# Kim-Dongjun/Soft-Truncation

Measured on AMD Instinct MI355X. Metric: training images/sec (DDPM++ CIFAR-10 32x32), higher is better.
Workload: dtype f32; 1 GPU; DDPM++ (VP) CIFAR-10 32x32, configs/vp/CIFAR10/ddpmpp_nll_st.py (BASELINE configs[1]); per_gpu_batch=128, global_batch=128, parallelism=dp1

## Files before the change

soft-truncation_amd/csrc/conv_x2w.h:

```cpp
#pragma once

namespace x2w {

typedef short s4 __attribute__((__vector_size__(8)));
typedef __attribute__((address_space(3))) s4 lds_s4;
typedef __attribute__((address_space(3))) void lds_void;

struct Args {
  const unsigned char* dypl; const float* dyrec; long dy_ps;
  const unsigned char* xpl; const float* xrec; long x_ps;
  float* part; long part_stride;
  int N, H, W, HW, Cin, Cout, Cob, Cib;
  int tiles_co, tiles_ci, nchunks_total, chunks_per_split;
};

__device__ __forceinline__ halfx8 cat(s4 lo, s4 hi) {
  typedef short s8 __attribute__((__vector_size__(16)));
  const s8 v = __builtin_shufflevector(lo, hi, 0, 1, 2, 3, 4, 5, 6, 7);
  return __builtin_bit_cast(halfx8, v);
}

constexpr int A_INSTR = 3;
constexpr int A_BLK = A_INSTR * 16 * 64;
constexpr int A_PLANE = 4 * A_BLK;
constexpr int B_INSTR = 6;
constexpr int B_PLANE = B_INSTR * 16 * 64;
constexpr int BUF = 2 * A_PLANE + 2 * B_PLANE;

constexpr int X1_FORM = 16;
template <int COLS, int FORM = 1>
__global__ __launch_bounds__(256 * (FORM & 15), 2) void wgrad_kernel(Args a) {
  constexpr int GROUPS = FORM & 15;
  constexpr bool X1 = (FORM & X1_FORM) != 0;
  constexpr int NS = X1 ? 1 : 2;
  constexpr int STAGES = 2;
  constexpr bool TWO = COLS == 4;
  constexpr int ROWS = 32 / COLS;
  constexpr int TPA = COLS + 2;
  constexpr int TRB = TWO ? 12 : ROWS + 2;
  constexpr int LDS = STAGES * BUF;
  static_assert(ROWS * TPA <= A_INSTR * 16 && TRB * COLS <= B_INSTR * 16, "tiles exceed the staged slots");
  __shared__ __attribute__((aligned(1024))) unsigned char lds_all[LDS * GROUPS];
  const int tid = threadIdx.x & 255, lane = tid & 63;
  const int grp = GROUPS == 1 ? 0 : __builtin_amdgcn_readfirstlane((int)threadIdx.x >> 8);
  const int wid = __builtin_amdgcn_readfirstlane(tid >> 6);
  unsigned char* const lds = lds_all + grp * LDS;
  __shared__ float red_amax[2][GROUPS][4];
  x2::LateAmax amax_dy, amax_x;
  amax_dy.load(a.dyrec, x2::NPART, tid);
  amax_x.load(a.xrec, x2::NPART, tid);
  const int ntiles = a.tiles_co * a.tiles_ci;
  const int id = xcd_remap(blockIdx.x, gridDim.x);
  const int tile = id % ntiles, zs = id / ntiles;
  const int tco = tile % a.tiles_co, tci = tile / a.tiles_co;
  const int co_blk = tco * 4 + wid;
  const bool co_live = co_blk < a.Cob;
  const int c_begin = zs * a.chunks_per_split;
  const int c_last = min(a.nchunks_total, c_begin + a.chunks_per_split) - 1;

  const __amdgpu_buffer_rsrc_t a_rs = x2::make_rsrc(a.dypl, 2L * a.dy_ps);
  const __amdgpu_buffer_rsrc_t b_rs = x2::make_rsrc(a.xpl, 2L * a.x_ps);
  const int piece = (lane & 3) * 16;
  int a_rel[A_INSTR], a_c[A_INSTR];
#pragma unroll
  for (int j = 0; j < A_INSTR; ++j) {
    const int sl = 16 * j + (lane >> 2);
    int r = sl / TPA;
    a_c[j] = sl - r * TPA;
    int img = 0;
    if (TWO) { img = r >> 2; r &= 3; }
    if (sl >= ROWS * TPA || !co_live) a_c[j] = -1000000;
    a_rel[j] = (img * a.Cob * a.HW + r * a.W + a_c[j] - 1) * 64 + piece;
  }
  int b_rel[3], b_ty[3], b_dst[3]; unsigned b_pl[3];
#pragma unroll
  for (int u = 0; u < 3; ++u) {
    const int idx = wid + 4 * u, j = idx % B_INSTR, pl = idx / B_INSTR;
    const int sl = 16 * j + (lane >> 2);
    b_ty[u] = sl / COLS;
    const int tx = sl - b_ty[u] * COLS;
    int img = 0;
    if (TWO) { img = b_ty[u] / 6; b_ty[u] -= 6 * img; }
    if (sl >= TRB * COLS) b_ty[u] = -1000000;
    b_rel[u] = (img * a.Cib * a.HW + (b_ty[u] - 1) * a.W + tx) * 64 + piece;
    b_dst[u] = 2 * A_PLANE + pl * B_PLANE + j * 1024;
    b_pl[u] = (unsigned)pl;
  }
  auto stage = [&](int c, unsigned char* buf) {
    const int p0 = c * 32;
    const int b = p0 / a.HW, hw0 = p0 - b * a.HW;
    const int y0 = hw0 / a.W, x0 = hw0 - y0 * a.W;
    const int a_chunk = ((b * a.Cob + co_blk) * a.HW + hw0) * 64;
#pragma unroll
    for (int j = 0; j < A_INSTR; ++j) {
      const int xx = x0 + a_c[j] - 1;
      const unsigned vo = (xx >= 0 && xx < a.W) ? (unsigned)(a_chunk + a_rel[j]) : 0x80000000u;
#pragma unroll
      for (int s = 0; s < NS; ++s)
        __builtin_amdgcn_raw_ptr_buffer_load_lds(a_rs, (lds_void*)(buf + s * A_PLANE + wid * A_BLK + j * 1024), 16,
                                                 (int)vo, (int)(s * (unsigned)a.dy_ps), 0, 0);
    }
    const int b_chunk = ((b * a.Cib + tci) * a.HW + hw0) * 64;
#pragma unroll
    for (int u = 0; u < 3; ++u) {
      if (X1 && b_pl[u]) continue;
      const int yy = y0 + b_ty[u] - 1;
      const unsigned vo = (yy >= 0 && yy < a.H) ? (unsigned)(b_chunk + b_rel[u]) : 0x80000000u;
      __builtin_amdgcn_raw_ptr_buffer_load_lds(b_rs, (lds_void*)(buf + b_dst[u]), 16, (int)vo, (int)(b_pl[u] * (unsigned)a.x_ps), 0, 0);
    }
  };

  floatx16 acc[9];
#pragma unroll
  for (int t = 0; t < 9; ++t)
#pragma unroll
    for (int e = 0; e < 16; ++e) acc[t][e] = 0.f;

  const int m = lane & 15, g = lane >> 4;
  const int ch_off = (16 * (g & 1) + 4 * (m & 3)) * 2;
  int a_off[2][2], b_off[2][2];
#pragma unroll
  for (int kk = 0; kk < 2; ++kk)
#pragma unroll
    for (int h = 0; h < 2; ++h) {
      const int k = 16 * kk + 8 * (g >> 1) + 4 * h + (m >> 2);
      const int krow = k / COLS, kcol = k - krow * COLS;
      a_off[kk][h] = wid * A_BLK + (krow * TPA + kcol + 1) * 64 + ch_off;
      const int trow = TWO ? (krow >> 2) * 6 + (krow & 3) : krow;
      b_off[kk][h] = 2 * A_PLANE + ((trow + 1) * COLS + kcol) * 64 + ch_off;
    }
  constexpr int SA[3] = {1, 0, 0}, SB[3] = {0, 1, 0};

  auto compute = [&](const unsigned char* buf) {
#pragma unroll
    for (int kk = 0; kk < 2; ++kk) {
      halfx8 af[3][2];
#pragma unroll
      for (int t = 0; t < 3; ++t)
#pragma unroll
        for (int s = 0; s < NS; ++s)
          af[t][s] = cat(__builtin_amdgcn_ds_read_tr16_b64_v4i16((lds_s4*)(buf + s * A_PLANE + a_off[kk][0] - (t - 1) * 64)),
                         __builtin_amdgcn_ds_read_tr16_b64_v4i16((lds_s4*)(buf + s * A_PLANE + a_off[kk][1] - (t - 1) * 64)));
#pragma unroll
      for (int t3 = 0; t3 < 3; ++t3) {
        halfx8 bf[2];
#pragma unroll
        for (int s = 0; s < NS; ++s)
          bf[s] = cat(__builtin_amdgcn_ds_read_tr16_b64_v4i16((lds_s4*)(buf + s * B_PLANE + b_off[kk][0] + (t3 - 1) * COLS * 64)),
                      __builtin_amdgcn_ds_read_tr16_b64_v4i16((lds_s4*)(buf + s * B_PLANE + b_off[kk][1] + (t3 - 1) * COLS * 64)));
#pragma unroll
        for (int pr = X1 ? 2 : 0; pr < 3; ++pr)
#pragma unroll
          for (int t = 0; t < 3; ++t)
            acc[3 * t3 + t] = __builtin_amdgcn_mfma_f32_32x32x16_f16(af[t][SA[pr]], bf[SB[pr]], acc[3 * t3 + t], 0, 0, 0);
      }
    }
  };

  const int rounds = (c_last - c_begin + GROUPS) / GROUPS;
#pragma unroll
  for (int i = 0; i < STAGES - 1; ++i)
    if (c_begin + i * GROUPS + grp <= c_last) stage(c_begin + i * GROUPS + grp, lds + i * BUF);
  int cur = 0;
  for (int it = 0; it < rounds; ++it) {
    const int c = c_begin + it * GROUPS + grp;
    asm volatile("s_waitcnt vmcnt(0)" ::: "memory");
    __syncthreads();
    const int nxt = cur + STAGES - 1 >= STAGES ? cur - 1 : cur + STAGES - 1;
    if (c + (STAGES - 1) * GROUPS <= c_last) stage(c + (STAGES - 1) * GROUPS, lds + nxt * BUF);
    if (c <= c_last) compute(lds + cur * BUF);
    cur = cur + 1 == STAGES ? 0 : cur + 1;
  }
  const float sa = x2::pow2_scale_of(amax_dy.reduce(red_amax[0][grp], tid));
  const float sb = x2::pow2_scale_of(amax_x.reduce(red_amax[1][grp], tid));
  const float unscale = 1.f / (sa * sb);
  if (GROUPS == 2) {
    float* const xch = reinterpret_cast<float*>(lds_all);
#pragma unroll
    for (int r = 0; r < 3; ++r) {
      __syncthreads();
      if (grp == 1) {
#pragma unroll
        for (int t = 0; t < 3; ++t)
#pragma unroll
          for (int e = 0; e < 16; ++e) xch[(16 * t + e) * 256 + tid] = acc[3 * r + t][e];
      }
      __syncthreads();
      if (grp == 0) {
#pragma unroll
        for (int t = 0; t < 3; ++t)
#pragma unroll
          for (int e = 0; e < 16; ++e) acc[3 * r + t][e] += xch[(16 * t + e) * 256 + tid];
      }
    }
    if (grp == 1) return;
  }

  float* slab = a.part + (long)zs * a.part_stride;
  const int fk = lane >> 5, fc = lane & 31;
  const int ci = tci * 32 + fc;
  if (co_live && ci < a.Cin) {
#pragma unroll
    for (int t = 0; t < 9; ++t)
#pragma unroll
      for (int e = 0; e < 16; ++e) {
        const int co = co_blk * 32 + 4 * fk + igemm::strip_row(e);
        if (co < a.Cout) slab[((long)t * a.Cout + co) * a.Cin + ci] = unscale * acc[t][e];
      }
  }
}


struct Plan { int ok; int splits; int chunks_per_split; long slab; int groups; };
inline int groups_mode() { static const int v = [] { const char* e = getenv("STK_X2W_GROUPS"); return e ? atoi(e) : 2; }(); return v; }
inline Plan plan(int N, int H, int W, int Cin, int Cout, int wgs = 0) {
  Plan r = {0, 1, 0, 0, 1};
  if (H != W || W < 4 || (W & (W - 1)) || Cin % 32 || Cout % 32 || Cin < 32 || Cout < 32) return r;
  const long px = (long)N * H * W;
  if (px % 32 || px / 32 > 0x7fffffffL / 64) return r;
  const int nch = (int)(px / 32);
  const long tiles = (long)stk_cdiv(Cout, 128) * (Cin / 32);
  static const long cap_mb = [] { const char* e = getenv("STK_WGRAD_SLAB_MB"); return e ? atol(e) : 128L; }();
  static const long shared = [] { const char* e = getenv("STK_X2W_WGS"); return e && atol(e) > 0 ? atol(e) : 256L; }();
  const long target = wgs > 0 ? wgs : shared;
  long splits = tiles >= target ? 1 : target / tiles;
  if (splits > nch / 8) splits = nch / 8;
  const long cap = (cap_mb << 20) / (9L * Cout * Cin * 4);
  if (splits > cap) splits = cap;
  if (splits < 1) splits = 1;
  const bool gw = groups_mode() == 3 || (groups_mode() == 2 && (W == 8 || W == 16));
  if (gw && splits >= 2 && splits % 2 == 0 && nch / splits >= 8) { r.groups = 2; splits /= 2; }
  r.chunks_per_split = stk_cdiv(nch, splits);
  r.splits = stk_cdiv(nch, r.chunks_per_split);
  r.slab = 9L * Cout * Cin;
  r.ok = nch >= 8;
  return r;
}

}
```

Measured before the change: 3438 images/s.

## Trim wgrad LDS staging: whole-row dy loads, exact x-tile instruction count, inline-asm DMA

Rewrites the LDS staging of the fp16 weight-gradient conv kernel. When dy tiles cover whole image rows, it issues two buffer-to-LDS loads instead of three and zeroes the halo columns once up front. It also issues only the x-tile load instructions that are actually live rather than a fixed three per wave. Buffer loads now go through inline asm that sets m0 directly, and lane/tid are recomputed late (mbcnt) to shorten live ranges. The aim is less redundant global traffic and lower VGPR pressure, at the cost of fragile hand-written asm (m0 save/restore, s_nop) and extra special-case index logic.

Result: faster. 3497 images/s (median of 6 runs) (+1.7%).

```diff
diff --git a/soft-truncation_amd/csrc/conv_x2w.h b/soft-truncation_amd/csrc/conv_x2w.h
--- a/soft-truncation_amd/csrc/conv_x2w.h
+++ b/soft-truncation_amd/csrc/conv_x2w.h
@@ -18,6 +18,17 @@
   typedef short s8 __attribute__((__vector_size__(16)));
   const s8 v = __builtin_shufflevector(lo, hi, 0, 1, 2, 3, 4, 5, 6, 7);
   return __builtin_bit_cast(halfx8, v);
+}
+
+__device__ __forceinline__ u32x4 rsrc_words(const void* base, long bytes) {
+  const unsigned long p = reinterpret_cast<unsigned long>(base);
+  return u32x4{(unsigned)p, (unsigned)(p >> 32) & 0xffffu, (unsigned)bytes, 0x00020000u};
+}
+__device__ __forceinline__ void dma16(u32x4 rs, const unsigned char* dst, unsigned voff, unsigned soff) {
+  const unsigned lds_addr = (unsigned)(unsigned long)(lds_void*)dst;
+  unsigned keep;
+  asm volatile("s_mov_b32 %0, m0\n\ts_mov_b32 m0, %1\n\ts_nop 4\n\tbuffer_load_dwordx4 %2, %3, %4 offen lds\n\ts_mov_b32 m0, %0"
+               : "=&s"(keep) : "s"(lds_addr), "v"(voff), "s"(rs), "s"(soff) : "memory");
 }
 
 constexpr int A_INSTR = 3;
@@ -58,10 +69,12 @@
   const int c_begin = zs * a.chunks_per_split;
   const int c_last = min(a.nchunks_total, c_begin + a.chunks_per_split) - 1;
 
-  const __amdgpu_buffer_rsrc_t a_rs = x2::make_rsrc(a.dypl, 2L * a.dy_ps);
-  const __amdgpu_buffer_rsrc_t b_rs = x2::make_rsrc(a.xpl, 2L * a.x_ps);
+  const u32x4 a_rs = rsrc_words(a.dypl, 2L * a.dy_ps);
+  const u32x4 b_rs = rsrc_words(a.xpl, 2L * a.x_ps);
   const int piece = (lane & 3) * 16;
-  int a_rel[A_INSTR], a_c[A_INSTR];
+  const bool a_whole_rows = COLS == 16 || (COLS == 32 && a.W == 32);
+  const int a_instr = a_whole_rows ? 2 : A_INSTR;
+  int a_rel[A_INSTR], a_c[A_INSTR], a_dst[A_INSTR];
 #pragma unroll
   for (int j = 0; j < A_INSTR; ++j) {
     const int sl = 16 * j + (lane >> 2);
@@ -69,15 +82,24 @@
     a_c[j] = sl - r * TPA;
     int img = 0;
     if (TWO) { img = r >> 2; r &= 3; }
-    if (sl >= ROWS * TPA || !co_live) a_c[j] = -1000000;
+    if (sl >= ROWS * TPA) a_c[j] = -1000000;
     a_rel[j] = (img * a.Cob * a.HW + r * a.W + a_c[j] - 1) * 64 + piece;
-  }
-  int b_rel[3], b_ty[3], b_dst[3]; unsigned b_pl[3];
-#pragma unroll
-  for (int u = 0; u < 3; ++u) {
-    const int idx = wid + 4 * u, j = idx % B_INSTR, pl = idx / B_INSTR;
+    a_dst[j] = wid * A_BLK + j * 1024;
+    if (a_whole_rows) {
+      a_c[j] = 1;
+      a_rel[j] = sl * 64 + piece;
+      a_dst[j] = wid * A_BLK + ((16 * j / COLS) * TPA + 16 * j % COLS + 1) * 64;
+    }
+    if (!co_live) { a_c[j] = -1000000; a_rel[j] = -1000000 * 64; }
+  }
+  constexpr int B_LIVE = TRB * COLS / 16, B_ALL = NS * B_LIVE, B_WAVE = (B_ALL + 3) / 4;
+  static_assert(B_LIVE * 16 == TRB * COLS && B_LIVE <= B_INSTR, "the x tile is whole instructions");
+  int b_rel[B_WAVE], b_ty[B_WAVE], b_dst[B_WAVE]; unsigned b_pl[B_WAVE];
+#pragma unroll
+  for (int u = 0; u < B_WAVE; ++u) {
+    const int idx = wid + 4 * u, j = idx % B_LIVE, pl = idx / B_LIVE;
     const int sl = 16 * j + (lane >> 2);
-    b_ty[u] = sl / COLS;
+    b_ty[u] = COLS >= 16 ? 16 * j / COLS : sl / COLS;
     const int tx = sl - b_ty[u] * COLS;
     int img = 0;
     if (TWO) { img = b_ty[u] / 6; b_ty[u] -= 6 * img; }
@@ -93,20 +115,21 @@
     const int a_chunk = ((b * a.Cob + co_blk) * a.HW + hw0) * 64;
 #pragma unroll
     for (int j = 0; j < A_INSTR; ++j) {
+      if (j >= a_instr) continue;
       const int xx = x0 + a_c[j] - 1;
-      const unsigned vo = (xx >= 0 && xx < a.W) ? (unsigned)(a_chunk + a_rel[j]) : 0x80000000u;
+      const bool in = COLS == 32 ? (unsigned)(x0 * 64 + a_rel[j]) < (unsigned)(a.W * 64) : (xx >= 0 && xx < a.W);
+      const unsigned vo = in ? (unsigned)(a_chunk + a_rel[j]) : 0x80000000u;
 #pragma unroll
       for (int s = 0; s < NS; ++s)
-        __builtin_amdgcn_raw_ptr_buffer_load_lds(a_rs, (lds_void*)(buf + s * A_PLANE + wid * A_BLK + j * 1024), 16,
-                                                 (int)vo, (int)(s * (unsigned)a.dy_ps), 0, 0);
+        dma16(a_rs, buf + s * A_PLANE + a_dst[j], vo, s * (unsigned)a.dy_ps);
     }
     const int b_chunk = ((b * a.Cib + tci) * a.HW + hw0) * 64;
 #pragma unroll
-    for (int u = 0; u < 3; ++u) {
-      if (X1 && b_pl[u]) continue;
+    for (int u = 0; u < B_WAVE; ++u) {
+      if (4 * u + 3 >= B_ALL && wid + 4 * u >= B_ALL) continue;
       const int yy = y0 + b_ty[u] - 1;
       const unsigned vo = (yy >= 0 && yy < a.H) ? (unsigned)(b_chunk + b_rel[u]) : 0x80000000u;
-      __builtin_amdgcn_raw_ptr_buffer_load_lds(b_rs, (lds_void*)(buf + b_dst[u]), 16, (int)vo, (int)(b_pl[u] * (unsigned)a.x_ps), 0, 0);
+      dma16(b_rs, buf + b_dst[u], vo, b_pl[u] * (unsigned)a.x_ps);
     }
   };
 
@@ -158,6 +181,14 @@
   };
 
   const int rounds = (c_last - c_begin + GROUPS) / GROUPS;
+  if (a_whole_rows) {
+    constexpr int NH = COLS >= 16 ? STAGES * NS * ROWS * 2 : 0;
+    static_assert(NH * 4 <= 64, "one store per lane");
+    const int h = lane >> 2, side = h & 1, r = (h >> 1) % ROWS, sp = (h >> 1) / ROWS;
+    if (h < NH)
+      *reinterpret_cast<uint4*>(lds + (sp / NS) * BUF + (sp % NS) * A_PLANE + wid * A_BLK + (r * TPA + side * (TPA - 1)) * 64 + piece) =
+          make_uint4(0u, 0u, 0u, 0u);
+  }
 #pragma unroll
   for (int i = 0; i < STAGES - 1; ++i)
     if (c_begin + i * GROUPS + grp <= c_last) stage(c_begin + i * GROUPS + grp, lds + i * BUF);
@@ -171,8 +202,10 @@
     if (c <= c_last) compute(lds + cur * BUF);
     cur = cur + 1 == STAGES ? 0 : cur + 1;
   }
-  const float sa = x2::pow2_scale_of(amax_dy.reduce(red_amax[0][grp], tid));
-  const float sb = x2::pow2_scale_of(amax_x.reduce(red_amax[1][grp], tid));
+  const int lane_late = (int)__builtin_amdgcn_mbcnt_hi(~0u, __builtin_amdgcn_mbcnt_lo(~0u, 0u));
+  const int tid_late = wid * 64 + lane_late;
+  const float sa = x2::pow2_scale_of(amax_dy.reduce(red_amax[0][grp], tid_late));
+  const float sb = x2::pow2_scale_of(amax_x.reduce(red_amax[1][grp], tid_late));
   const float unscale = 1.f / (sa * sb);
   if (GROUPS == 2) {
     float* const xch = reinterpret_cast<float*>(lds_all);
@@ -183,21 +216,21 @@
 #pragma unroll
         for (int t = 0; t < 3; ++t)
 #pragma unroll
-          for (int e = 0; e < 16; ++e) xch[(16 * t + e) * 256 + tid] = acc[3 * r + t][e];
+          for (int e = 0; e < 16; ++e) xch[(16 * t + e) * 256 + tid_late] = acc[3 * r + t][e];
       }
       __syncthreads();
       if (grp == 0) {
 #pragma unroll
         for (int t = 0; t < 3; ++t)
 #pragma unroll
-          for (int e = 0; e < 16; ++e) acc[3 * r + t][e] += xch[(16 * t + e) * 256 + tid];
+          for (int e = 0; e < 16; ++e) acc[3 * r + t][e] += xch[(16 * t + e) * 256 + tid_late];
       }
     }
     if (grp == 1) return;
   }
 
   float* slab = a.part + (long)zs * a.part_stride;
-  const int fk = lane >> 5, fc = lane & 31;
+  const int fk = lane_late >> 5, fc = lane_late & 31;
   const int ci = tci * 32 + fc;
   if (co_live && ci < a.Cin) {
 #pragma unroll
```
